# joyfang1106/MRLA

Hardware: AMD Instinct MI355X
Metric: images/sec fwd+bwd resnet50_mrlal b=256 (higher is better)
Workload: dtype bf16

## Files before the change

### mrla_amd/csrc/conv_spatial.h

```cpp
#pragma once
#include <algorithm>

#include "conv1x1_elem.h"
#include "mrla_device.h"
#include "mrla_kernels.h"

namespace mrla {
namespace {

typedef short tr_s16x4 __attribute__((ext_vector_type(4)));
typedef __attribute__((address_space(3))) tr_s16x4* tr_lds_s16x4_ptr;

constexpr int kTileRowB = 128;

__device__ __forceinline__ tr_s16x4 tr16_read(const unsigned char* p) {
  return __builtin_amdgcn_ds_read_tr16_b64_v4i16((tr_lds_s16x4_ptr)p);
}
template <typename T>
__device__ __forceinline__ typename Elem16<T>::x8 tr16_frag(const unsigned char* lo_ptr, const unsigned char* hi_ptr) {
  return __builtin_bit_cast(typename Elem16<T>::x8, __builtin_shufflevector(tr16_read(lo_ptr), tr16_read(hi_ptr), 0, 1, 2, 3, 4, 5, 6, 7));
}

template <int MASK, int SHIFT>
__device__ __forceinline__ int tile_off(int row, int chunk) {
  return row * kTileRowB + ((chunk ^ (((row >> 1) & MASK) << SHIFT)) << 4);
}

__device__ __forceinline__ int tr_krel(int lane) {
  const int g = lane >> 4, q = (lane >> 2) & 3;
  return 8 * (g >> 1) + q;
}
__device__ __forceinline__ int tr_col(int block, int lane) {
  const int g = lane >> 4, pp = lane & 3;
  return block + 16 * (g & 1) + 4 * pp;
}
__device__ __forceinline__ int tr_chunk(int col) { return col >> 3; }
__device__ __forceinline__ int tr_sub(int col) { return ((col >> 2) & 1) * 8; }

struct RowStep {
  int img, yo0, R;
};
__device__ __forceinline__ RowStep row_step(int r, int r_end, int ho, int rmax) {
  RowStep s;
  s.img = r / ho;
  s.yo0 = r - s.img * ho;
  s.R = min(rmax, min(ho - s.yo0, r_end - r));
  return s;
}

template <typename TO>
__global__ __launch_bounds__(256) void split_sum_kernel(const float* __restrict__ part, TO* __restrict__ dW, int splits,
                                                        int total4) {
  const int i = blockIdx.x * 256 + threadIdx.x;
  if (i >= total4) return;
  const float4* src = reinterpret_cast<const float4*>(part) + i;
  float4 s = src[0];
#pragma unroll 8
  for (int k = 1; k < splits; ++k) {
    const float4 v = src[(size_t)k * total4];
    s.x += v.x; s.y += v.y; s.z += v.z; s.w += v.w;
  }
  TO* o = dW + (size_t)i * 4;
  o[0] = from_f<TO>(s.x); o[1] = from_f<TO>(s.y); o[2] = from_f<TO>(s.z); o[3] = from_f<TO>(s.w);
}

template <typename = void>
int launch_split_sum(const float* part, void* dw, int dw_f32, int dtype, int splits, int total, hipStream_t st) {
  const int total4 = total / 4;
  const dim3 grid((total4 + 255) / 256), block(256);
  if (dw_f32)
    hipLaunchKernelGGL(split_sum_kernel<float>, grid, block, 0, st, part, (float*)dw, splits, total4);
  else if (dtype == MRLA_F16)
    hipLaunchKernelGGL(split_sum_kernel<f16_t>, grid, block, 0, st, part, (f16_t*)dw, splits, total4);
  else
    hipLaunchKernelGGL(split_sum_kernel<bf16_t>, grid, block, 0, st, part, (bf16_t*)dw, splits, total4);
  return hip_status(hipGetLastError());
}

struct Raster3x3 {
  int ok = 0;
  int ho = 0, wo = 0;
  int py = 0, ws = 0, nseg = 0, rmax = 0;
  int kp_cap = 0, xt_cap = 0;
};
static inline Raster3x3 raster3x3(int b, int c, int n, int h, int w, int s, int max_kp1, int max_kp2, int max_py, int kp_round) {
  Raster3x3 p;
  if (b <= 0 || c <= 0 || n <= 0 || h <= 0 || w <= 0 || (s != 1 && s != 2) || c % 64 || n % 64) return p;
  if ((unsigned long long)b * h * w * std::max(c, n) * 2 >= 1ull << 31) return p;
  p.ho = (h - 1) / s + 1;
  p.wo = (w - 1) / s + 1;
  const int pad = s == 1 ? 2 : 1;
  if (p.wo + pad <= max_py) {
    p.ws = p.wo; p.py = p.wo + pad; p.nseg = 1;
    p.rmax = std::max(1, std::min(p.ho, (s == 1 ? max_kp1 : max_kp2) / p.py));
  } else {
    p.py = max_py; p.ws = max_py - pad; p.nseg = (p.wo + p.ws - 1) / p.ws;
    p.rmax = 1;
  }
  p.kp_cap = (p.rmax * p.py + kp_round - 1) & ~(kp_round - 1);
  p.xt_cap = (s * p.kp_cap + s * (s - 1) * p.py * (p.rmax - 1) + 2 * s * p.py + 3 + 7) & ~7;
  p.ok = 1;
  return p;
}

struct RowSplit {
  int per, count;
};
static inline RowSplit split_rows(long long rows, int tiles, int target, long long floor_rows = 1, long long min_per = 1) {
  const long long want = std::max<long long>(1, std::min<long long>(rows / floor_rows, (target + tiles - 1) / tiles));
  RowSplit r;
  r.per = (int)std::max<long long>((rows + want - 1) / want, min_per);
  r.count = (int)((rows + r.per - 1) / r.per);
  return r;
}

}
}
```

### mrla_amd/csrc/stem_wgrad.hip

```cpp
#include <algorithm>

#include "conv_spatial.h"

namespace mrla {
namespace {

typedef c1_f32x16 sw_f32x16;

constexpr int kSwTile = 64;
constexpr int kSwWaves = 4;
constexpr int kSwBlocks = 3;
static_assert(2 * kSwBlocks * 32 >= 7 * 24, "the waves' blocks cover the 7 x 24 columns");
constexpr int kSwTarget = 2 * 256;
constexpr int kSwMaxWS = 128;
constexpr int kSwMaxKP = 256;
constexpr int kSwMaxR = 16;
static_assert(kSwMaxKP == 8 * 32 && kSwMaxWS <= kSwMaxKP, "the dY loader takes the tile in one pass");
static_assert(kTileRowB == kSwTile * 2, "a dY tile row is one pixel, 64 channels");
constexpr int kSwLdsCap = 64 * 1024;

struct SwPlan {
  int ok = 0;
  int ho = 0, wo = 0;
  int ws = 0, nseg = 0, rmax = 0;
  int kp_cap = 0, pd = 0, lds = 0;
  int rows_per_split = 0, splits = 0, tiles = 0;
};

struct SwArgs {
  int b, h, w, ho, wo, n;
  int ws, nseg, rmax, kp_cap, pd;
  int rows_per_split, splits;
  float inv_ws, inv_runs;
};

__device__ __forceinline__ int sw_off(int row, int chunk) { return tile_off<1, 2>(row, chunk); }

template <typename T>
__global__ __launch_bounds__(kSwWaves* kWave, 2) void stem_wgrad_kernel(const T* __restrict__ dY, const T* __restrict__ X,
                                                                        float* __restrict__ part, SwArgs a) {
#if defined(__HIP_DEVICE_COMPILE__)
  extern __shared__ __align__(16) unsigned char smem_raw[];
  unsigned char* const ty_tile = smem_raw;
  unsigned char* const tx_rows = smem_raw + a.kp_cap * kTileRowB;
  const int tid = threadIdx.x, lane = tid & (kWave - 1), wave = tid / kWave;
  const int tiles = a.n / kSwTile;
  const int split = blockIdx.x / tiles, tn = blockIdx.x - split * tiles;
  const int n0 = tn * kSwTile;
  const int rows = a.b * a.ho;
  const int r_begin = split * a.rows_per_split, r_end = min(rows, r_begin + a.rows_per_split);
  const int copyB = a.pd * 4, rowB = 2 * copyB;

  const int wn = wave >> 1, wc = wave & 1;
  const int krel = tr_krel(lane);
  const int colA = tr_col(wn * 32, lane);
  const int chA = tr_chunk(colA), subA = tr_sub(colA);
  int offB[kSwBlocks];
#pragma unroll
  for (int bl = 0; bl < kSwBlocks; ++bl) {
    const int col = tr_col(32 * (kSwBlocks * wc + bl), lane);
    const int kh = min(col / 24, 6), j = col % 24;
    offB[bl] = kh * rowB + 2 * j;
  }

  sw_f32x16 acc[kSwBlocks];
#pragma unroll
  for (int t = 0; t < kSwBlocks; ++t)
#pragma unroll
    for (int e = 0; e < 16; ++e) acc[t][e] = 0.f;

  const int prow = tid >> 3, pch = tid & 7;
  const u32x4 zero4 = {0u, 0u, 0u, 0u};
  const int runs = a.pd / 4 - 1;
  const bool even_w = (a.w & 1) == 0;
  const int row_el = 3 * a.w;
  const uint32_t* const Xd = reinterpret_cast<const uint32_t*>(X);
  const unsigned short* const Xe = reinterpret_cast<const unsigned short*>(X);

  for (int r = r_begin; r < r_end;) {
    const RowStep st = row_step(r, r_end, a.ho, a.rmax);
    const int img = st.img, yo0 = st.yo0, R = st.R;
    for (int seg = 0; seg < a.nseg; ++seg) {
      const int xo0 = seg * a.ws, ws = min(a.ws, a.wo - xo0);
      const int NP = R * ws, KP = (NP + 15) & ~15;
      const int XR = 2 * R + 5;
      const int yi0 = 2 * yo0 - 3;
      __syncthreads();
      u32x4 v[8];
#pragma unroll
      for (int u = 0; u < 8; ++u) {
        const int p = 32 * u + prow;
        const int ry = (int)(((float)p + 0.5f) * a.inv_ws), xl = p - ry * a.ws;
        v[u] = zero4;
        if (p < KP && ry < R && xl < ws)
          v[u] = *reinterpret_cast<const u32x4*>(dY + ((size_t)((img * a.ho + yo0 + ry) * a.wo + xo0 + xl) * a.n + n0 + pch * 8));
      }
      const int nrun = XR * runs;
      auto load_run = [&](int idx, uint32_t (&raw)[8]) {
        const int t = (int)(((float)idx + 0.5f) * a.inv_runs), m = idx - t * runs;
        const int yi = yi0 + t;
        const bool row_ok = idx < nrun && yi >= 0 && yi < a.h;
        const int row0 = (img * a.h + yi) * row_el;
        if (even_w) {
          const int g0 = 3 * xo0 - 5 + 4 * m, ndw = row_el >> 1;
#pragma unroll
          for (int i = 0; i < 5; ++i) {
            const int gi = g0 + i;
            raw[i] = 0u;
            if (row_ok && gi >= 0 && gi < ndw) raw[i] = Xd[(row0 >> 1) + gi];
          }
        } else {
          const int e0 = 6 * xo0 - 9 + 8 * m;
#pragma unroll
          for (int i = 0; i < 8; ++i) {
            const int ei = e0 + i;
            raw[i] = 0u;
            if (row_ok && ei >= 0 && ei < row_el) raw[i] = Xe[row0 + ei];
          }
        }
      };
      auto store_run = [&](int idx, const uint32_t (&raw)[8]) {
        if (idx >= nrun) return;
        const int t = (int)(((float)idx + 0.5f) * a.inv_runs), m = idx - t * runs;
        uint32_t d[4];
#pragma unroll
        for (int i = 0; i < 4; ++i) d[i] = even_w ? (raw[i] >> 16) | (raw[i + 1] << 16) : raw[2 * i] | (raw[2 * i + 1] << 16);
        unsigned char* const ra = tx_rows + t * rowB + 16 * m;
        *reinterpret_cast<u32x4*>(ra) = u32x4{d[0], d[1], d[2], d[3]};
        uint32_t* const rb = reinterpret_cast<uint32_t*>(ra + copyB + 4);
        rb[0] = d[0]; rb[1] = d[1]; rb[2] = d[2]; rb[3] = d[3];
      };
      constexpr int kThreadsWg = kSwWaves * kWave;
      uint32_t x0[8], x1[8];
      load_run(tid, x0);
      load_run(tid + kThreadsWg, x1);
#pragma unroll
      for (int u = 0; u < 8; ++u) {
        const int p = 32 * u + prow;
        if (p < KP) *reinterpret_cast<u32x4*>(ty_tile + sw_off(p, pch)) = v[u];
      }
      store_run(tid, x0);
      store_run(tid + kThreadsWg, x1);
      for (int idx = tid + 2 * kThreadsWg; idx < nrun; idx += 2 * kThreadsWg) {
        load_run(idx, x0);
        load_run(idx + kThreadsWg, x1);
        store_run(idx, x0);
        store_run(idx + kThreadsWg, x1);
      }
      __syncthreads();
      for (int k0 = 0; k0 < KP; k0 += 16) {
        const int k = k0 + krel;
        const typename Elem16<T>::x8 fa = tr16_frag<T>(ty_tile + sw_off(k, chA) + subA, ty_tile + sw_off(k + 4, chA) + subA);
        const int p1 = min(k, NP - 1), p2 = min(k + 4, NP - 1);
        const int ry1 = (int)(((float)p1 + 0.5f) * a.inv_ws), xl1 = p1 - ry1 * a.ws;
        const int ry2 = (int)(((float)p2 + 0.5f) * a.inv_ws), xl2 = p2 - ry2 * a.ws;
        const unsigned char* const b1 = tx_rows + 2 * ry1 * rowB + 12 * xl1 + (xl1 & 1) * (copyB + 4);
        const unsigned char* const b2 = tx_rows + 2 * ry2 * rowB + 12 * xl2 + (xl2 & 1) * (copyB + 4);
#pragma unroll
        for (int bl = 0; bl < kSwBlocks; ++bl) {
          const typename Elem16<T>::x8 fb = tr16_frag<T>(b1 + offB[bl], b2 + offB[bl]);
          Elem16<T>::mfma(acc[bl], fa, fb);
        }
      }
    }
    r += R;
  }

  const int hh = lane >> 5;
#pragma unroll
  for (int bl = 0; bl < kSwBlocks; ++bl) {
    const int col = 32 * (kSwBlocks * wc + bl) + (lane & 31);
    const int kh = col / 24, j = col - kh * 24;
    if (kh < 7 && j < 21) {
      float* po = part + ((size_t)split * a.n + n0 + wn * 32) * 147 + kh * 21 + j;
#pragma unroll
      for (int e = 0; e < 16; ++e) po[(size_t)(8 * (e >> 2) + 4 * hh + (e & 3)) * 147] = acc[bl][e];
    }
  }
#endif
}

SwPlan sw_plan(int b, int n, int h, int w) {
  SwPlan p;
  if (b <= 0 || n <= 0 || h <= 0 || w <= 0 || n % kSwTile) return p;
  if ((unsigned long long)b * h * w * std::max(3, n) * 2 >= 1ull << 31) return p;
  p.ho = (h - 1) / 2 + 1;
  p.wo = (w - 1) / 2 + 1;
  if (p.wo <= kSwMaxWS) {
    p.ws = p.wo; p.nseg = 1;
    p.rmax = std::max(1, std::min(std::min(p.ho, kSwMaxR), kSwMaxKP / p.ws));
  } else {
    p.ws = kSwMaxWS; p.nseg = (p.wo + p.ws - 1) / p.ws;
    p.rmax = 1;
  }
  p.kp_cap = (p.rmax * p.ws + 15) & ~15;
  const int ew = (6 * p.ws + 18 + 7) & ~7;
  p.pd = ew / 2 + 4;
  p.lds = p.kp_cap * kTileRowB + (2 * p.rmax + 5) * 2 * p.pd * 4;
  if (p.lds > kSwLdsCap) return p;
  p.tiles = n / kSwTile;
  const long long rows = (long long)b * p.ho;
  const RowSplit sp = split_rows(rows, p.tiles, kSwTarget, 1, std::min<long long>(rows, p.rmax));
  p.rows_per_split = sp.per;
  p.splits = sp.count;
  p.ok = 1;
  return p;
}

template <typename T>
int sw_launch(const SwPlan& p, const SwArgs& a, const void* dy, const void* x, float* part, hipStream_t st) {
  if (lds_opt_in(reinterpret_cast<const void*>(stem_wgrad_kernel<T>), (size_t)p.lds) != hipSuccess) return MRLA_EHIP;
  hipLaunchKernelGGL((stem_wgrad_kernel<T>), dim3(p.tiles * p.splits), dim3(kSwWaves * kWave), (size_t)p.lds, st, (const T*)dy,
                     (const T*)x, part, a);
  return MRLA_OK;
}

}

int stem_conv_wgrad_rows(int b, int n, int h, int w) {
  const SwPlan p = sw_plan(b, n, h, w);
  return p.ok ? p.splits : MRLA_EUNSUPPORTED;
}

int stem_conv_wgrad_plan(int b, int n, int h, int w, int* out) {
  const SwPlan p = sw_plan(b, n, h, w);
  if (!p.ok) return MRLA_EUNSUPPORTED;
  out[0] = kSwTile; out[1] = p.rows_per_split; out[2] = p.splits; out[3] = p.nseg; out[4] = p.lds; out[5] = p.ws; out[6] = p.rmax;
  return MRLA_OK;
}

int launch_stem_conv_wgrad(const void* dy, const void* x, float* part, void* dw, int dw_f32, int b, int n, int h, int w,
                           int dtype, hipStream_t st) {
  const SwPlan p = sw_plan(b, n, h, w);
  if (!p.ok || (dtype != MRLA_BF16 && dtype != MRLA_F16)) return MRLA_EUNSUPPORTED;
  SwArgs a;
  a.b = b; a.h = h; a.w = w; a.ho = p.ho; a.wo = p.wo; a.n = n;
  a.ws = p.ws; a.nseg = p.nseg; a.rmax = p.rmax; a.kp_cap = p.kp_cap; a.pd = p.pd;
  a.rows_per_split = p.rows_per_split; a.splits = p.splits;
  a.inv_ws = 1.0f / (float)p.ws; a.inv_runs = 1.0f / (float)(p.pd / 4 - 1);
  const int rc = dtype == MRLA_F16 ? sw_launch<f16_t>(p, a, dy, x, part, st) : sw_launch<bf16_t>(p, a, dy, x, part, st);
  if (rc != MRLA_OK) return rc;
  return launch_split_sum(part, dw, dw_f32, dtype, p.splits, n * 147, st);
}

}
```

Baseline: 9277.

## Prefetch next stem wgrad segment during MFMA loop and widen-adapt split-sum reduction

Result: no change. 9209 (-0.7%).

```diff
diff --git a/mrla_amd/csrc/conv_spatial.h b/mrla_amd/csrc/conv_spatial.h
--- a/mrla_amd/csrc/conv_spatial.h
+++ b/mrla_amd/csrc/conv_spatial.h
@@ -48,32 +48,55 @@
   return s;
 }
 
+template <typename TO, int V, int U>
+__device__ __forceinline__ void split_sum_lane(const float* __restrict__ part, TO* __restrict__ dW, int splits, int total, int i) {
+  typedef float vec __attribute__((ext_vector_type(V)));
+  const float* src = part + (size_t)i * V;
+  vec s = *reinterpret_cast<const vec*>(src);
+  int k = 1;
+  for (; k + U <= splits; k += U) {
+    vec v[U];
+#pragma unroll
+    for (int u = 0; u < U; ++u) v[u] = *reinterpret_cast<const vec*>(src + (size_t)(k + u) * total);
+#pragma unroll
+    for (int u = 0; u < U; ++u) s += v[u];
+  }
+  for (; k < splits; ++k) s += *reinterpret_cast<const vec*>(src + (size_t)k * total);
+  TO* o = dW + (size_t)i * V;
+#pragma unroll
+  for (int e = 0; e < V; ++e) o[e] = from_f<TO>(s[e]);
+}
+
 template <typename TO>
 __global__ __launch_bounds__(256) void split_sum_kernel(const float* __restrict__ part, TO* __restrict__ dW, int splits,
-                                                        int total4) {
-  const int i = blockIdx.x * 256 + threadIdx.x;
-  if (i >= total4) return;
-  const float4* src = reinterpret_cast<const float4*>(part) + i;
-  float4 s = src[0];
-#pragma unroll 8
-  for (int k = 1; k < splits; ++k) {
-    const float4 v = src[(size_t)k * total4];
-    s.x += v.x; s.y += v.y; s.z += v.z; s.w += v.w;
-  }
-  TO* o = dW + (size_t)i * 4;
-  o[0] = from_f<TO>(s.x); o[1] = from_f<TO>(s.y); o[2] = from_f<TO>(s.z); o[3] = from_f<TO>(s.w);
+                                                        int total, int width) {
+  const int i = blockIdx.x * blockDim.x + threadIdx.x;
+  if (i >= total / width) return;
+  if (width == 4)
+    split_sum_lane<TO, 4, 8>(part, dW, splits, total, i);
+  else if (width == 2)
+    split_sum_lane<TO, 2, 16>(part, dW, splits, total, i);
+  else
+    split_sum_lane<TO, 1, 32>(part, dW, splits, total, i);
+}
+
+constexpr int kSumCUs = 256, kSumWavesPerCU = 2;
+static inline int split_sum_width(int total) {
+  const int want = kSumCUs * kSumWavesPerCU * kWave;
+  return total / 4 >= want ? 4 : total / 2 >= want ? 2 : 1;
 }
 
 template <typename = void>
 int launch_split_sum(const float* part, void* dw, int dw_f32, int dtype, int splits, int total, hipStream_t st) {
-  const int total4 = total / 4;
-  const dim3 grid((total4 + 255) / 256), block(256);
+  const int width = split_sum_width(total), lanes = total / width;
+  const int threads = width == 4 ? 256 : kWave;
+  const dim3 grid((lanes + threads - 1) / threads), block(threads);
   if (dw_f32)
-    hipLaunchKernelGGL(split_sum_kernel<float>, grid, block, 0, st, part, (float*)dw, splits, total4);
+    hipLaunchKernelGGL(split_sum_kernel<float>, grid, block, 0, st, part, (float*)dw, splits, total, width);
   else if (dtype == MRLA_F16)
-    hipLaunchKernelGGL(split_sum_kernel<f16_t>, grid, block, 0, st, part, (f16_t*)dw, splits, total4);
+    hipLaunchKernelGGL(split_sum_kernel<f16_t>, grid, block, 0, st, part, (f16_t*)dw, splits, total, width);
   else
-    hipLaunchKernelGGL(split_sum_kernel<bf16_t>, grid, block, 0, st, part, (bf16_t*)dw, splits, total4);
+    hipLaunchKernelGGL(split_sum_kernel<bf16_t>, grid, block, 0, st, part, (bf16_t*)dw, splits, total, width);
   return hip_status(hipGetLastError());
 }
 
diff --git a/mrla_amd/csrc/stem_wgrad.hip b/mrla_amd/csrc/stem_wgrad.hip
--- a/mrla_amd/csrc/stem_wgrad.hip
+++ b/mrla_amd/csrc/stem_wgrad.hip
@@ -18,6 +18,7 @@
 static_assert(kSwMaxKP == 8 * 32 && kSwMaxWS <= kSwMaxKP, "the dY loader takes the tile in one pass");
 static_assert(kTileRowB == kSwTile * 2, "a dY tile row is one pixel, 64 channels");
 constexpr int kSwLdsCap = 64 * 1024;
+constexpr int kSwPreRuns = 4;
 
 struct SwPlan {
   int ok = 0;
@@ -76,94 +77,140 @@
   const int row_el = 3 * a.w;
   const uint32_t* const Xd = reinterpret_cast<const uint32_t*>(X);
   const unsigned short* const Xe = reinterpret_cast<const unsigned short*>(X);
-
-  for (int r = r_begin; r < r_end;) {
+  constexpr int kThreadsWg = kSwWaves * kWave;
+
+  struct Seg {
+    int r, seg, img, yo0, R, xo0, ws;
+  };
+  auto seg_at = [&](int r, int seg) {
     const RowStep st = row_step(r, r_end, a.ho, a.rmax);
-    const int img = st.img, yo0 = st.yo0, R = st.R;
-    for (int seg = 0; seg < a.nseg; ++seg) {
-      const int xo0 = seg * a.ws, ws = min(a.ws, a.wo - xo0);
-      const int NP = R * ws, KP = (NP + 15) & ~15;
-      const int XR = 2 * R + 5;
-      const int yi0 = 2 * yo0 - 3;
-      __syncthreads();
-      u32x4 v[8];
-#pragma unroll
-      for (int u = 0; u < 8; ++u) {
-        const int p = 32 * u + prow;
+    Seg g;
+    g.r = r; g.seg = seg; g.img = st.img; g.yo0 = st.yo0; g.R = st.R;
+    g.xo0 = seg * a.ws; g.ws = min(a.ws, a.wo - g.xo0);
+    return g;
+  };
+  auto load_y = [&](const Seg& g, u32x4 (&v)[8]) {
+    const int KP = (g.R * g.ws + 15) & ~15;
+#pragma unroll
+    for (int u = 0; u < 8; ++u) {
+      int p = 32 * u + prow;
+      v[u] = zero4;
+      if (p < KP) {
+        asm volatile("" : "+v"(p));
         const int ry = (int)(((float)p + 0.5f) * a.inv_ws), xl = p - ry * a.ws;
-        v[u] = zero4;
-        if (p < KP && ry < R && xl < ws)
-          v[u] = *reinterpret_cast<const u32x4*>(dY + ((size_t)((img * a.ho + yo0 + ry) * a.wo + xo0 + xl) * a.n + n0 + pch * 8));
-      }
-      const int nrun = XR * runs;
-      auto load_run = [&](int idx, uint32_t (&raw)[8]) {
-        const int t = (int)(((float)idx + 0.5f) * a.inv_runs), m = idx - t * runs;
-        const int yi = yi0 + t;
-        const bool row_ok = idx < nrun && yi >= 0 && yi < a.h;
-        const int row0 = (img * a.h + yi) * row_el;
-        if (even_w) {
-          const int g0 = 3 * xo0 - 5 + 4 * m, ndw = row_el >> 1;
-#pragma unroll
-          for (int i = 0; i < 5; ++i) {
-            const int gi = g0 + i;
-            raw[i] = 0u;
-            if (row_ok && gi >= 0 && gi < ndw) raw[i] = Xd[(row0 >> 1) + gi];
-          }
-        } else {
-          const int e0 = 6 * xo0 - 9 + 8 * m;
-#pragma unroll
-          for (int i = 0; i < 8; ++i) {
-            const int ei = e0 + i;
-            raw[i] = 0u;
-            if (row_ok && ei >= 0 && ei < row_el) raw[i] = Xe[row0 + ei];
-          }
+        if (ry < g.R && xl < g.ws)
+          v[u] = *reinterpret_cast<const u32x4*>(dY + ((size_t)((g.img * a.ho + g.yo0 + ry) * a.wo + g.xo0 + xl) * a.n + n0 + pch * 8));
+      }
+    }
+  };
+  auto load_run_even = [&](const Seg& g, int idx, uint32_t (&raw)[5]) {
+#pragma unroll
+    for (int i = 0; i < 5; ++i) raw[i] = 0u;
+    if (idx < (2 * g.R + 5) * runs) {
+      asm volatile("" : "+v"(idx));
+      const int t = (int)(((float)idx + 0.5f) * a.inv_runs), m = idx - t * runs;
+      const int yi = 2 * g.yo0 - 3 + t;
+      if (yi >= 0 && yi < a.h) {
+        const int g0 = 3 * g.xo0 - 5 + 4 * m, ndw = row_el >> 1;
+        const uint32_t* const row = Xd + (((g.img * a.h + yi) * row_el) >> 1);
+#pragma unroll
+        for (int i = 0; i < 5; ++i) {
+          const int gi = g0 + i;
+          if (gi >= 0 && gi < ndw) raw[i] = row[gi];
         }
-      };
-      auto store_run = [&](int idx, const uint32_t (&raw)[8]) {
-        if (idx >= nrun) return;
-        const int t = (int)(((float)idx + 0.5f) * a.inv_runs), m = idx - t * runs;
-        uint32_t d[4];
-#pragma unroll
-        for (int i = 0; i < 4; ++i) d[i] = even_w ? (raw[i] >> 16) | (raw[i + 1] << 16) : raw[2 * i] | (raw[2 * i + 1] << 16);
-        unsigned char* const ra = tx_rows + t * rowB + 16 * m;
-        *reinterpret_cast<u32x4*>(ra) = u32x4{d[0], d[1], d[2], d[3]};
-        uint32_t* const rb = reinterpret_cast<uint32_t*>(ra + copyB + 4);
-        rb[0] = d[0]; rb[1] = d[1]; rb[2] = d[2]; rb[3] = d[3];
-      };
-      constexpr int kThreadsWg = kSwWaves * kWave;
-      uint32_t x0[8], x1[8];
-      load_run(tid, x0);
-      load_run(tid + kThreadsWg, x1);
-#pragma unroll
-      for (int u = 0; u < 8; ++u) {
-        const int p = 32 * u + prow;
-        if (p < KP) *reinterpret_cast<u32x4*>(ty_tile + sw_off(p, pch)) = v[u];
-      }
-      store_run(tid, x0);
-      store_run(tid + kThreadsWg, x1);
-      for (int idx = tid + 2 * kThreadsWg; idx < nrun; idx += 2 * kThreadsWg) {
-        load_run(idx, x0);
-        load_run(idx + kThreadsWg, x1);
-        store_run(idx, x0);
-        store_run(idx + kThreadsWg, x1);
-      }
-      __syncthreads();
-      for (int k0 = 0; k0 < KP; k0 += 16) {
-        const int k = k0 + krel;
-        const typename Elem16<T>::x8 fa = tr16_frag<T>(ty_tile + sw_off(k, chA) + subA, ty_tile + sw_off(k + 4, chA) + subA);
-        const int p1 = min(k, NP - 1), p2 = min(k + 4, NP - 1);
-        const int ry1 = (int)(((float)p1 + 0.5f) * a.inv_ws), xl1 = p1 - ry1 * a.ws;
-        const int ry2 = (int)(((float)p2 + 0.5f) * a.inv_ws), xl2 = p2 - ry2 * a.ws;
-        const unsigned char* const b1 = tx_rows + 2 * ry1 * rowB + 12 * xl1 + (xl1 & 1) * (copyB + 4);
-        const unsigned char* const b2 = tx_rows + 2 * ry2 * rowB + 12 * xl2 + (xl2 & 1) * (copyB + 4);
-#pragma unroll
-        for (int bl = 0; bl < kSwBlocks; ++bl) {
-          const typename Elem16<T>::x8 fb = tr16_frag<T>(b1 + offB[bl], b2 + offB[bl]);
-          Elem16<T>::mfma(acc[bl], fa, fb);
-        }
-      }
-    }
-    r += R;
+      }
+    }
+  };
+  auto load_run_odd = [&](const Seg& g, int idx, uint32_t (&raw)[8]) {
+    const int t = (int)(((float)idx + 0.5f) * a.inv_runs), m = idx - t * runs;
+    const int yi = 2 * g.yo0 - 3 + t;
+    const bool row_ok = idx < (2 * g.R + 5) * runs && yi >= 0 && yi < a.h;
+    const int row0 = (g.img * a.h + yi) * row_el;
+    const int e0 = 6 * g.xo0 - 9 + 8 * m;
+#pragma unroll
+    for (int i = 0; i < 8; ++i) {
+      const int ei = e0 + i;
+      raw[i] = 0u;
+      if (row_ok && ei >= 0 && ei < row_el) raw[i] = Xe[row0 + ei];
+    }
+  };
+  auto store_run = [&](int nrun, int idx, const uint32_t (&d)[4]) {
+    if (idx >= nrun) return;
+    const int t = (int)(((float)idx + 0.5f) * a.inv_runs), m = idx - t * runs;
+    unsigned char* const ra = tx_rows + t * rowB + 16 * m;
+    *reinterpret_cast<u32x4*>(ra) = u32x4{d[0], d[1], d[2], d[3]};
+    uint32_t* const rb = reinterpret_cast<uint32_t*>(ra + copyB + 4);
+    rb[0] = d[0]; rb[1] = d[1]; rb[2] = d[2]; rb[3] = d[3];
+  };
+  auto store_run_even = [&](int nrun, int idx, const uint32_t (&raw)[5]) {
+    uint32_t d[4];
+#pragma unroll
+    for (int i = 0; i < 4; ++i) d[i] = (raw[i] >> 16) | (raw[i + 1] << 16);
+    store_run(nrun, idx, d);
+  };
+  auto store_run_odd = [&](int nrun, int idx, const uint32_t (&raw)[8]) {
+    uint32_t d[4];
+#pragma unroll
+    for (int i = 0; i < 4; ++i) d[i] = raw[2 * i] | (raw[2 * i + 1] << 16);
+    store_run(nrun, idx, d);
+  };
+
+  u32x4 vy[8];
+  uint32_t vx[kSwPreRuns][5];
+  auto prefetch = [&](const Seg& g) {
+    load_y(g, vy);
+    if (even_w) {
+#pragma unroll
+      for (int j = 0; j < kSwPreRuns; ++j) load_run_even(g, tid + j * kThreadsWg, vx[j]);
+    }
+  };
+  Seg cur = seg_at(r_begin, 0);
+  bool more = r_begin < r_end;
+  if (more) prefetch(cur);
+  while (more) {
+    const int R = cur.R;
+    const int NP = R * cur.ws, KP = (NP + 15) & ~15;
+    const int nrun = (2 * R + 5) * runs;
+    __syncthreads();
+#pragma unroll
+    for (int u = 0; u < 8; ++u) {
+      const int p = 32 * u + prow;
+      if (p < KP) *reinterpret_cast<u32x4*>(ty_tile + sw_off(p, pch)) = vy[u];
+    }
+    if (even_w) {
+#pragma unroll
+      for (int j = 0; j < kSwPreRuns; ++j) store_run_even(nrun, tid + j * kThreadsWg, vx[j]);
+    } else {
+      for (int idx = tid; idx < nrun; idx += 2 * kThreadsWg) {
+        uint32_t x0[8], x1[8];
+        load_run_odd(cur, idx, x0);
+        load_run_odd(cur, idx + kThreadsWg, x1);
+        store_run_odd(nrun, idx, x0);
+        store_run_odd(nrun, idx + kThreadsWg, x1);
+      }
+    }
+    __syncthreads();
+    Seg nxt = cur;
+    more = cur.seg + 1 < a.nseg || cur.r + R < r_end;
+    if (more) {
+      nxt = cur.seg + 1 < a.nseg ? seg_at(cur.r, cur.seg + 1) : seg_at(cur.r + R, 0);
+      prefetch(nxt);
+    }
+    for (int k0 = 0; k0 < KP; k0 += 16) {
+      const int k = k0 + krel;
+      const typename Elem16<T>::x8 fa = tr16_frag<T>(ty_tile + sw_off(k, chA) + subA, ty_tile + sw_off(k + 4, chA) + subA);
+      const int p1 = min(k, NP - 1), p2 = min(k + 4, NP - 1);
+      const int ry1 = (int)(((float)p1 + 0.5f) * a.inv_ws), xl1 = p1 - ry1 * a.ws;
+      const int ry2 = (int)(((float)p2 + 0.5f) * a.inv_ws), xl2 = p2 - ry2 * a.ws;
+      const unsigned char* const b1 = tx_rows + 2 * ry1 * rowB + 12 * xl1 + (xl1 & 1) * (copyB + 4);
+      const unsigned char* const b2 = tx_rows + 2 * ry2 * rowB + 12 * xl2 + (xl2 & 1) * (copyB + 4);
+#pragma unroll
+      for (int bl = 0; bl < kSwBlocks; ++bl) {
+        const typename Elem16<T>::x8 fb = tr16_frag<T>(b1 + offB[bl], b2 + offB[bl]);
+        Elem16<T>::mfma(acc[bl], fa, fb);
+      }
+    }
+    cur = nxt;
   }
 
   const int hh = lane >> 5;
@@ -198,6 +245,7 @@
   p.pd = ew / 2 + 4;
   p.lds = p.kp_cap * kTileRowB + (2 * p.rmax + 5) * 2 * p.pd * 4;
   if (p.lds > kSwLdsCap) return p;
+  if ((2 * p.rmax + 5) * (p.pd / 4 - 1) > kSwPreRuns * kSwWaves * kWave) return p;
   p.tiles = n / kSwTile;
   const long long rows = (long long)b * p.ho;
   const RowSplit sp = split_rows(rows, p.tiles, kSwTarget, 1, std::min<long long>(rows, p.rmax));
```
